# tier4/icp_rust

Hardware: AMD Instinct MI355X
Metric: ICP iterations/sec on 1M-pt 3D pair (higher is better)
Workload: dtype f64

## Files before the change

icp_rust_amd/csrc/gn_device.hpp:

```cpp
#pragma once
#include "common.hpp"

namespace icp {

__device__ __forceinline__ unsigned long long f2k(double v) {
  const unsigned long long u = (unsigned long long)__double_as_longlong(v);
  return (u >> 63) ? ~u : (u | 0x8000000000000000ull);
}
__device__ __forceinline__ double k2f(unsigned long long k) {
  const unsigned long long u = (k >> 63) ? (k & 0x7fffffffffffffffull) : ~k;
  return __longlong_as_double((long long)u);
}

__device__ __forceinline__ int pass_shift(int pass) { return pass < 5 ? 52 - 12 * pass : 0; }
__device__ __forceinline__ int pass_bits(int pass) { return pass < 5 ? 12 : 4; }

__device__ __forceinline__ double huber_rho(double e) {
  const double k = ICP_HUBER_K;
  const double k2 = k * k;
  return (e <= k2) ? e : (2. * k * __dsqrt_rn(e) - k2);
}
__device__ __forceinline__ double huber_drho(double e) {
  const double k = ICP_HUBER_K;
  const double k2 = k * k;
  return (e <= k2) ? 1. : (k / __dsqrt_rn(e));
}

__device__ __forceinline__ unsigned wave_scan_inclusive(unsigned v) {
#define ICP_SCAN_DPP(x, ctrl, rows) (unsigned)__builtin_amdgcn_update_dpp(0, (int)(x), ctrl, rows, 0xf, true)
  v += ICP_SCAN_DPP(v, 0x111, 0xf);
  v += ICP_SCAN_DPP(v, 0x112, 0xf);
  v += ICP_SCAN_DPP(v, 0x114, 0xf);
  v += ICP_SCAN_DPP(v, 0x118, 0xf);
  v += ICP_SCAN_DPP(v, 0x142, 0xa);
  v += ICP_SCAN_DPP(v, 0x143, 0xc);
#undef ICP_SCAN_DPP
  return v;
}

template <int OFF>
__device__ __forceinline__ double tree_down(double v) {
  if constexpr (OFF >= 16) {
#ifdef ICP_TREE_BPERMUTE
    return __shfl_down(v, OFF);
#else
    const long long b = __double_as_longlong(v);
    const unsigned lo = (unsigned)(b & 0xffffffffll), hi = (unsigned)((unsigned long long)b >> 32);
    if constexpr (OFF == 32) {
      const auto rl = __builtin_amdgcn_permlane32_swap(lo, lo, false, false);
      const auto rh = __builtin_amdgcn_permlane32_swap(hi, hi, false, false);
      return __longlong_as_double((long long)(((unsigned long long)rh[1] << 32) | rl[1]));
    } else {
      const auto rl = __builtin_amdgcn_permlane16_swap(lo, lo, false, false);
      const auto rh = __builtin_amdgcn_permlane16_swap(hi, hi, false, false);
      return __longlong_as_double((long long)(((unsigned long long)rh[1] << 32) | rl[1]));
    }
#endif
  } else {
    const long long b = __double_as_longlong(v);
    const int lo = __builtin_amdgcn_update_dpp(0, (int)(b & 0xffffffffll), 0x100 + OFF, 0xf, 0xf, true);
    const int hi = __builtin_amdgcn_update_dpp(0, (int)(b >> 32), 0x100 + OFF, 0xf, 0xf, true);
    return __longlong_as_double(((long long)hi << 32) | (unsigned)lo);
  }
}
template <int N, int OFF>
__device__ __forceinline__ void tree_step(double (&acc)[N]) {
  double t[N];
#pragma unroll
  for (int k = 0; k < N; ++k) t[k] = tree_down<OFF>(acc[k]);
#pragma unroll
  for (int k = 0; k < N; ++k) acc[k] = acc[k] + t[k];
}
template <int N>
__device__ __forceinline__ void wave_tree(double (&acc)[N]) {
  tree_step<N, 32>(acc);
  tree_step<N, 16>(acc);
  tree_step<N, 8>(acc);
  tree_step<N, 4>(acc);
  tree_step<N, 2>(acc);
  tree_step<N, 1>(acc);
}

template <int N>
__device__ __forceinline__ void block_reduce_waves(double (&acc)[N], double (*sm)[N]) {
  wave_tree<N>(acc);
  if ((threadIdx.x & 63) == 0) {
#pragma unroll
    for (int k = 0; k < N; ++k) sm[threadIdx.x >> 6][k] = acc[k];
  }
}
template <int N, bool SC1 = false>
__device__ __forceinline__ void block_reduce_finish(const double (*sm)[N], double *__restrict__ out) {
  if (threadIdx.x < N) {
    const int k = threadIdx.x;
    double s = sm[0][k];
    for (int w = 1; w < (int)(blockDim.x >> 6); ++w) s = s + sm[w][k];
    if (SC1) __hip_atomic_store(out + k, s, __ATOMIC_RELAXED, __HIP_MEMORY_SCOPE_AGENT);
    else out[k] = s;
  }
}
template <int N, bool SC1 = false>
__device__ __forceinline__ void block_reduce_store(double (&acc)[N], double *__restrict__ out) {
  __shared__ double sm[16][N];
  block_reduce_waves<N>(acc, sm);
  __syncthreads();
  block_reduce_finish<N, SC1>(sm, out);
}


__device__ __forceinline__ bool last_block_arrives(TicketSet *t) {
  __shared__ int s_last;
  asm volatile("s_waitcnt vmcnt(0)" ::: "memory");
  __syncthreads();
  if (threadIdx.x == 0) {
    const unsigned nb = gridDim.x, sh = blockIdx.x & 15u;
    const unsigned in_shard = (nb - sh + 15u) >> 4;
    int last = 0;
    if (nb <= 32u) {
      if (__hip_atomic_fetch_add(&t->top[0], 1u, __ATOMIC_RELAXED, __HIP_MEMORY_SCOPE_AGENT) == nb - 1) {
        __hip_atomic_store(&t->top[0], 0u, __ATOMIC_RELAXED, __HIP_MEMORY_SCOPE_AGENT);
        last = 1;
      }
    } else if (__hip_atomic_fetch_add(&t->shard[sh][0], 1u, __ATOMIC_RELAXED, __HIP_MEMORY_SCOPE_AGENT) == in_shard - 1) {
      __hip_atomic_store(&t->shard[sh][0], 0u, __ATOMIC_RELAXED, __HIP_MEMORY_SCOPE_AGENT);
      const unsigned nshards = nb < 16u ? nb : 16u;
      if (__hip_atomic_fetch_add(&t->top[0], 1u, __ATOMIC_RELAXED, __HIP_MEMORY_SCOPE_AGENT) == nshards - 1) {
        __hip_atomic_store(&t->top[0], 0u, __ATOMIC_RELAXED, __HIP_MEMORY_SCOPE_AGENT);
        last = 1;
      }
    }
    s_last = last;
  }
  __syncthreads();
  return s_last != 0;
}

template <bool UNIFORM>
__device__ __forceinline__ void accumulate_dim(int j, const double2 &s, double r_j, const Pose &T, double *S) {
  const double k2 = ICP_HUBER_K * ICP_HUBER_K;
  const double a0 = -s.y, a1 = s.x;
  const double J0 = j ? T.r10 : T.r00, J1 = j ? T.r11 : T.r01;
  const double J2 = J0 * a0 + J1 * a1;
  const double e = r_j * r_j;
  double w = 1.;
  if (UNIFORM) {
    if (__ballot(e > k2)) w = huber_drho(e);
  } else {
    w = huber_drho(e);
  }
  const double t0 = w * J0, t1 = w * J1, t2 = w * J2;
  S[0] = S[0] + t0 * J0;
  S[1] = S[1] + t0 * J1;
  S[2] = S[2] + t0 * J2;
  S[3] = S[3] + t1 * J1;
  S[4] = S[4] + t1 * J2;
  S[5] = S[5] + t2 * J2;
  S[6] = S[6] + t0 * r_j;
  S[7] = S[7] + t1 * r_j;
  S[8] = S[8] + t2 * r_j;
}

template <bool UNIFORM>
__device__ __forceinline__ void accumulate_rho(double r0, double r1, double *err) {
  const double k2 = ICP_HUBER_K * ICP_HUBER_K;
  const double e2 = r0 * r0 + r1 * r1;
  double rho = e2;
  if (UNIFORM) {
    if (__ballot(e2 > k2)) rho = huber_rho(e2);
  } else {
    rho = huber_rho(e2);
  }
  *err = *err + rho;
}

__device__ __forceinline__ void accumulate_dim_w(int j, const double2 &s, double r_j, double w, const Pose &T, double *S) {
  const double a0 = -s.y, a1 = s.x;
  const double J0 = j ? T.r10 : T.r00, J1 = j ? T.r11 : T.r01;
  const double J2 = J0 * a0 + J1 * a1;
  const double t0 = w * J0, t1 = w * J1, t2 = w * J2;
  S[0] = S[0] + t0 * J0;
  S[1] = S[1] + t0 * J1;
  S[2] = S[2] + t0 * J2;
  S[3] = S[3] + t1 * J1;
  S[4] = S[4] + t1 * J2;
  S[5] = S[5] + t2 * J2;
  S[6] = S[6] + t0 * r_j;
  S[7] = S[7] + t1 * r_j;
  S[8] = S[8] + t2 * r_j;
}

template <bool UNIFORM>
__device__ __forceinline__ void accumulate_pair(const double2 &s, double r0, double r1, const Pose &T, double *acc) {
  if constexpr (UNIFORM) {
    const double k2 = ICP_HUBER_K * ICP_HUBER_K;
    const double e0 = r0 * r0, e1 = r1 * r1, e2 = e0 + e1;
    double w0 = 1., w1 = 1., rho = e2;
    if (__ballot((e0 > k2) | (e1 > k2) | (e2 > k2))) {
      w0 = huber_drho(e0);
      w1 = huber_drho(e1);
      rho = huber_rho(e2);
    }
    accumulate_dim_w(0, s, r0, w0, T, acc);
    accumulate_dim_w(1, s, r1, w1, T, acc + 9);
    acc[18] = acc[18] + rho;
  } else {
    accumulate_dim<UNIFORM>(0, s, r0, T, acc);
    accumulate_dim<UNIFORM>(1, s, r1, T, acc + 9);
    accumulate_rho<UNIFORM>(r0, r1, acc + 18);
  }
}

__host__ __device__ __forceinline__ double combine_sum(const double *S, int k, const double *sig) {
  if (k >= 12) return S[18];
  int u;
  if (k >= 9) {
    u = 6 + (k - 9);
  } else {
    const int p = k / 3, q = k % 3;
    const int lo = p < q ? p : q, hi = p < q ? q : p;
    u = lo == 0 ? hi : (lo == 1 ? 2 + hi : 5);
  }
  double v = 0.;
  if (sig[0] != 0.) v = v + (1. / sig[0]) * S[u];
  if (sig[1] != 0.) v = v + (1. / sig[1]) * S[9 + u];
  return v;
}

__device__ __forceinline__ void accumulate_points(const double2 *__restrict__ a, const double *__restrict__ rx,
                                                  const double *__restrict__ ry, unsigned n, const Pose &T,
                                                  double (&acc)[kNSum]) {
  constexpr int kAccBatch = 4;
  const unsigned G = gridDim.x * kReduceThreads;
  for (unsigned base = blockIdx.x * kReduceThreads + threadIdx.x; base < n; base += G * kAccBatch) {
    double2 s[kAccBatch];
    double r0[kAccBatch], r1[kAccBatch];
#pragma unroll
    for (int u = 0; u < kAccBatch; ++u) {
      const unsigned i = base + u * G;
      if (i < n) {
        s[u] = a[i];
        r0[u] = rx[i];
        r1[u] = ry[i];
      }
    }
#pragma unroll
    for (int u = 0; u < kAccBatch; ++u) {
      const unsigned i = base + u * G;
      if (i >= n) continue;
      accumulate_pair<true>(s[u], r0[u], r1[u], T, acc);
    }
  }
}

template <int SCOPE = __HIP_MEMORY_SCOPE_AGENT>
__device__ __forceinline__ void fold_block_sums(const double *partials, int blocks, double *s_tot) {
  double tot[kNSum + 1];
#pragma unroll
  for (int k = 0; k < kNSum + 1; ++k) tot[k] = 0.;
  for (int i = threadIdx.x; i < blocks; i += kReduceThreads) {
    double v[kNSum];
#pragma unroll
    for (int k = 0; k < kNSum; ++k)
      v[k] = __hip_atomic_load(&partials[(size_t)i * (kNSum + 1) + k], __ATOMIC_RELAXED, SCOPE);
#pragma unroll
    for (int k = 0; k < kNSum; ++k) tot[k] = tot[k] + v[k];
  }
  block_reduce_store<kNSum + 1>(tot, s_tot);
}

template <int SCOPE = __HIP_MEMORY_SCOPE_AGENT>
__device__ __forceinline__ void fold_block_sums_lean(const double *partials, int blocks, double *s_tot) {
  __shared__ double sm[kReduceThreads / 64];
  const int t = threadIdx.x;
  for (int q = 0; q < kNSum; ++q) {
    double v[1] = {0.};
    for (int i = t; i < blocks; i += kReduceThreads)
      v[0] = v[0] + __hip_atomic_load(&partials[(size_t)i * (kNSum + 1) + q], __ATOMIC_RELAXED, SCOPE);
    wave_tree<1>(v);
    if ((t & 63) == 0) sm[t >> 6] = v[0];
    __syncthreads();
    if (t == 0) {
      double s = sm[0];
      for (int w = 1; w < kReduceThreads / 64; ++w) s = s + sm[w];
      s_tot[q] = s;
    }
    __syncthreads();
  }
  if (t == 0) s_tot[kNSum] = 0.;
  __syncthreads();
}

constexpr int kFoldH = (kNSum + 1) / 2;
template <int SCOPE = __HIP_MEMORY_SCOPE_AGENT>
__device__ __forceinline__ void fold256_load(const double *partials, int blocks, double (&x)[kFoldH]) {
  static_assert(kReduceThreads == 512 && (kNSum + 1) == 20 && kReduceMaxBlocks <= 256, "two halves of ten sums, one row per thread");
  const int t = threadIdx.x, row = t & 255, half = t >> 8;
#pragma unroll
  for (int k = 0; k < kFoldH; ++k)
    x[k] = (row < blocks && half * kFoldH + k < kNSum)
               ? __hip_atomic_load(&partials[(size_t)row * (kNSum + 1) + half * kFoldH + k], __ATOMIC_RELAXED, SCOPE)
               : 0.;
}
__device__ __forceinline__ void fold256_reduce(const double (&x)[kFoldH], int blocks, double *s_tot) {
  constexpr int H = kFoldH;
  __shared__ double sm[8][H];
  const int t = threadIdx.x, row = t & 255, lane = t & 63, wave = t >> 6;
  double v[H];
#pragma unroll
  for (int k = 0; k < H; ++k) v[k] = 0.;
  if (row < blocks) {
#pragma unroll
    for (int k = 0; k < H; ++k) v[k] = v[k] + x[k];
  }
  wave_tree<H>(v);
  if (lane == 0) {
#pragma unroll
    for (int k = 0; k < H; ++k) sm[wave][k] = v[k];
  }
  __syncthreads();
  if (t < kNSum + 1) {
    const int h = t / H, k = t % H;
    double s = sm[4 * h][k];
    for (int w = 1; w < 4; ++w) s = s + sm[4 * h + w][k];
    s_tot[t] = s + 0.;
  }
}
constexpr int kFoldQ = kFoldH / 2;
template <int SCOPE = __HIP_MEMORY_SCOPE_AGENT>
__device__ __forceinline__ void fold256_half_load(const double *partials, int blocks, int h, double (&x)[kFoldQ]) {
  static_assert(kFoldQ * 2 == kFoldH, "two quarters per half");
  const int t = threadIdx.x, row = t & 255, c0 = h * kFoldH + (t >> 8) * kFoldQ;
#pragma unroll
  for (int k = 0; k < kFoldQ; ++k)
    x[k] = (row < blocks && c0 + k < kNSum)
               ? __hip_atomic_load(&partials[(size_t)row * (kNSum + 1) + c0 + k], __ATOMIC_RELAXED, SCOPE)
               : 0.;
}
__device__ __forceinline__ void fold256_half_reduce(const double (&x)[kFoldQ], int blocks, double *out) {
  constexpr int Q = kFoldQ;
  __shared__ double sm[8][Q];
  const int t = threadIdx.x, row = t & 255, lane = t & 63, wave = t >> 6;
  double v[Q];
#pragma unroll
  for (int k = 0; k < Q; ++k) v[k] = 0.;
  if (row < blocks) {
#pragma unroll
    for (int k = 0; k < Q; ++k) v[k] = v[k] + x[k];
  }
  wave_tree<Q>(v);
  if (lane == 0) {
#pragma unroll
    for (int k = 0; k < Q; ++k) sm[wave][k] = v[k];
  }
  __syncthreads();
  if (t < kFoldH) {
    const int g = t / Q, k = t % Q;
    double s = sm[4 * g][k];
    for (int w = 1; w < 4; ++w) s = s + sm[4 * g + w][k];
    out[t] = s + 0.;
  }
}

template <int SCOPE = __HIP_MEMORY_SCOPE_AGENT>
__device__ __forceinline__ void fold_block_sums_256(const double *partials, int blocks, double *s_tot) {
  double x[kFoldH];
  fold256_load<SCOPE>(partials, blocks, x);
  fold256_reduce(x, blocks, s_tot);
}

template <int SCOPE = __HIP_MEMORY_SCOPE_AGENT>
__device__ __forceinline__ double fold_one_load(const double *partials, int blocks, int q) {
  const int t = threadIdx.x;
  return (t < 256 && t < blocks && q < kNSum) ? __hip_atomic_load(&partials[(size_t)t * (kNSum + 1) + q], __ATOMIC_RELAXED, SCOPE)
                                               : 0.;
}
__device__ __forceinline__ double fold_one_reduce(double x, int blocks, double *sm4) {
  const int t = threadIdx.x, lane = t & 63, wave = t >> 6;
  double v[1] = {0.};
  if (t < 256 && t < blocks) v[0] = v[0] + x;
  wave_tree<1>(v);
  if (t < 256 && lane == 0) sm4[wave] = v[0];
  __syncthreads();
  double s = sm4[0];
  for (int w = 1; w < 4; ++w) s = s + sm4[w];
  return s + 0.;
}
template <int SCOPE = __HIP_MEMORY_SCOPE_AGENT>
__device__ __forceinline__ double fold_one_sum_256(const double *partials, int blocks, int q, double *sm4) {
  const int t = threadIdx.x, lane = t & 63, wave = t >> 6;
  double v[1] = {0.};
  if (t < 256) {
    const double x = (t < blocks && q < kNSum) ? __hip_atomic_load(&partials[(size_t)t * (kNSum + 1) + q], __ATOMIC_RELAXED, SCOPE) : 0.;
    if (t < blocks) v[0] = v[0] + x;
  }
  wave_tree<1>(v);
  if (t < 256 && lane == 0) sm4[wave] = v[0];
  __syncthreads();
  double s = sm4[0];
  for (int w = 1; w < 4; ++w) s = s + sm4[w];
  return s + 0.;
}

__device__ __forceinline__ void publish_folded(const double *s_tot, GnResult *res, unsigned seq, const double (&sig)[2],
                                               const double (&med)[2], int nan_flag, int overflow) {
  if (threadIdx.x < 64) {
    if (threadIdx.x < kNAcc + 1)
      res->acc[threadIdx.x] = threadIdx.x < kNAcc ? combine_sum(s_tot, (int)threadIdx.x, sig) : 0.;
    if (threadIdx.x == kNAcc + 1) {
      res->sigma[0] = sig[0];
      res->sigma[1] = sig[1];
      res->median[0] = med[0];
      res->median[1] = med[1];
    }
    if (threadIdx.x == kNAcc + 2) {
      res->nan_flag = nan_flag;
      res->overflow = overflow;
    }
    asm volatile("s_waitcnt vmcnt(0)" ::: "memory");
    if (threadIdx.x == 0) __hip_atomic_store(&res->seq, seq, __ATOMIC_RELEASE, __HIP_MEMORY_SCOPE_SYSTEM);
  }
}

template <int W>
__device__ __forceinline__ void publish_values(const double *s_tot, GnResult *res, const double (&sig)[2],
                                               const double (&med)[2], int nan_flag, int overflow) {
  const int t = (int)threadIdx.x - 64 * W;
  if (t >= 0 && t < 64) {
    if (t < kNAcc + 1) res->acc[t] = t < kNAcc ? combine_sum(s_tot, t, sig) : 0.;
    if (t == kNAcc + 1) {
      res->sigma[0] = sig[0];
      res->sigma[1] = sig[1];
      res->median[0] = med[0];
      res->median[1] = med[1];
    }
    if (t == kNAcc + 2) {
      res->nan_flag = nan_flag;
      res->overflow = overflow;
    }
    asm volatile("s_waitcnt vmcnt(0)" ::: "memory");
  }
}
__device__ __forceinline__ void publish_seq(GnResult *res, unsigned seq) {
  if (threadIdx.x < 64) {
    asm volatile("s_waitcnt vmcnt(0)" ::: "memory");
    if (threadIdx.x == 0) __hip_atomic_store(&res->seq, seq, __ATOMIC_RELEASE, __HIP_MEMORY_SCOPE_SYSTEM);
  }
}

__device__ __forceinline__ void publish_result(const double *partials, GnResult *res, unsigned seq,
                                               const double (&sig)[2], const double (&med)[2], int nan_flag,
                                               int overflow, int blocks_override = 0) {
  __shared__ double s_tot[kNSum + 1];
  fold_block_sums(partials, blocks_override > 0 ? blocks_override : (int)gridDim.x, s_tot);
  __syncthreads();
  publish_folded(s_tot, res, seq, sig, med, nan_flag, overflow);
}

}
```

Measured before the change: 10330.

## Use packed permlane swaps to fold paired accumulators in wave reduction

Replaces the per-accumulator butterfly reduction for the first two stages with permlane32/permlane16 swap-based folds that combine two accumulators per exchange, halving the lane-exchange work at each of those stages. After these two folds each 16-lane quarter holds a different subset of the sums. The remaining steps reduce a quarter as many values, and the lanes at 16-lane boundaries write their results to interleaved shared-memory slots. This relies on gfx950 permlane swap builtins and adds index bookkeeping that could misplace sums if the lane mapping is wrong.

```diff
diff --git a/icp_rust_amd/csrc/gn_device.hpp b/icp_rust_amd/csrc/gn_device.hpp
--- a/icp_rust_amd/csrc/gn_device.hpp
+++ b/icp_rust_amd/csrc/gn_device.hpp
@@ -81,8 +81,52 @@
   tree_step<N, 1>(acc);
 }
 
+#ifndef ICP_TREE_BPERMUTE
+template <bool P32>
+__device__ __forceinline__ double packed_fold(double x, double y) {
+  const long long bx = __double_as_longlong(x), by = __double_as_longlong(y);
+  const unsigned xl = (unsigned)(bx & 0xffffffffll), xh = (unsigned)((unsigned long long)bx >> 32);
+  const unsigned yl = (unsigned)(by & 0xffffffffll), yh = (unsigned)((unsigned long long)by >> 32);
+  unsigned Xl, Xh, Yl, Yh;
+  if constexpr (P32) {
+    const auto rl = __builtin_amdgcn_permlane32_swap(xl, yl, false, false);
+    const auto rh = __builtin_amdgcn_permlane32_swap(xh, yh, false, false);
+    Xl = rl[0], Yl = rl[1], Xh = rh[0], Yh = rh[1];
+  } else {
+    const auto rl = __builtin_amdgcn_permlane16_swap(xl, yl, false, false);
+    const auto rh = __builtin_amdgcn_permlane16_swap(xh, yh, false, false);
+    Xl = rl[0], Yl = rl[1], Xh = rh[0], Yh = rh[1];
+  }
+  const double X = __longlong_as_double((long long)(((unsigned long long)Xh << 32) | Xl));
+  const double Y = __longlong_as_double((long long)(((unsigned long long)Yh << 32) | Yl));
+  return X + Y;
+}
+#endif
 template <int N>
 __device__ __forceinline__ void block_reduce_waves(double (&acc)[N], double (*sm)[N]) {
+#ifndef ICP_TREE_BPERMUTE
+  if constexpr (N >= 4) {
+    constexpr int M1 = (N + 1) / 2, M2 = (M1 + 1) / 2;
+    double p[M1], q[M2];
+#pragma unroll
+    for (int j = 0; j < N / 2; ++j) p[j] = packed_fold<true>(acc[2 * j], acc[2 * j + 1]);
+    if constexpr (N & 1) p[M1 - 1] = acc[N - 1] + tree_down<32>(acc[N - 1]);
+#pragma unroll
+    for (int j = 0; j < M1 / 2; ++j) q[j] = packed_fold<false>(p[2 * j], p[2 * j + 1]);
+    if constexpr (M1 & 1) q[M2 - 1] = p[M1 - 1] + tree_down<16>(p[M1 - 1]);
+    tree_step<M2, 8>(q);
+    tree_step<M2, 4>(q);
+    tree_step<M2, 2>(q);
+    tree_step<M2, 1>(q);
+    if ((threadIdx.x & 15) == 0) {
+      const int r = (threadIdx.x >> 4) & 3, c = 2 * (r & 1) + (r >> 1);
+#pragma unroll
+      for (int j = 0; j < M2; ++j)
+        if (4 * j + c < N) sm[threadIdx.x >> 6][4 * j + c] = q[j];
+    }
+    return;
+  }
+#endif
   wave_tree<N>(acc);
   if ((threadIdx.x & 63) == 0) {
 #pragma unroll
```

Result: faster. 10430 (median of 6 runs) (+1.0%).
